# kabachuha/sd-webui-text2video

Measured on AMD Instinct MI355X. Metric: denoised frames/sec (UNet+VAE), ModelScope 24f@256x256, higher is better.
Workload: dtype f16; 1 GPU; ModelScope t2v fp16 (random-init 1.41B UNetSD + VAE decoder), 24 frames @ 256x256, 50 DDIM_Gaussian steps, CFG 9.0 (BASELINE.json configs[1]); one step = one whole video; frames_per_video=24, videos_per_batch=1, layout=single, layout_requested=auto, parallelism=1 GPU: cond+uncond batched as b=2

## Files before the change

sd-webui-text2video_amd/csrc/executor.hip:

```cpp
#include <hip/hip_runtime.h>

#include <cstdio>
#include <cstdlib>
#include <cstring>
#include <initializer_list>
#include <string>
#include <type_traits>
#include <vector>

#include "t2v_kernels.h"

namespace {

thread_local std::string g_err;

int fail(int code, const std::string& msg) {
  g_err = msg;
  return code;
}

inline bool resolve_ptrs(t2v_op& op, const uint64_t* ext, int n_ext) {
  for (int k = 0; k < T2V_OP_NP; ++k) {
    const uint64_t v = op.p[k];
    if (v != 0 && v < T2V_EXT_SLOTS) {
      if ((int)v >= n_ext || ext == nullptr) return false;
      op.p[k] = ext[v];
    }
  }
  return true;
}

enum GemmForm {
  GEMM_MALFORMED,
  GEMM_PLAIN, GEMM_GEGLU,
  GEMM_STATS,
  GEMM_LN_ROW, GEMM_LN_CROSS,
  GEMM_GN_TILE, GEMM_GN_SPLITK,
  GEMM_TATTN, GEMM_XATTN,
};
inline bool gemm_writes_gn(GemmForm f) { return f == GEMM_GN_TILE || f == GEMM_GN_SPLITK; }
struct GemmView {
  GemmForm form;
  const char* why;
  const t2v_tile* tile;
  int M, N, K, lda, ldw, ldc, ldr, ldrb;
  int gather, epi, act, out_dtype, out_item, split, bias_m, halo, rows_per_batch;
  int Hin, Win, Cin, stride, up, Hout, Wout, F, HW, tpix;
  int ln_mode, ld_ln;
  int hilo, out_lo;
  int res_wrap, a_wrap;
  int64_t n_out;
  int gn_rows, ld_gn, gn_silu, gn_lo, gn_groups, gn_skip_out;
  int xa_ldk, xa_lc, xa_lcp, xa_k_sample, xa_vt_sample;
  float ln_eps, attn_scale, gn_eps;
  bool waive_min_m;
  uint64_t A, W, bias, rowbias, ln_gb, res, out, ws;
  uint64_t tickets, ln_out, stats;
  uint64_t gn_gb, gn_out, xa_k, xa_vt;
  uint64_t scratch, barrier;
};

GemmView gemm_decode(const t2v_op& op) {
  const int32_t* I = op.i;
  const uint64_t* P = op.p;
  GemmView v;
  memset(&v, 0, sizeof v);
  const int M = v.M = I[0], N = v.N = I[1], K = v.K = I[2], g = v.gather = I[7], epi = v.epi = I[16];
  const bool plain = g == T2V_GATHER_PLAIN, conv = g == T2V_GATHER_CONV3X3 || g == T2V_GATHER_CONV3X3_C8;
  v.lda = I[3]; v.ldw = I[4]; v.ldc = I[5]; v.ldr = I[6]; v.ldrb = I[21];
  v.act = I[18]; v.out_dtype = I[17]; v.out_item = I[17] == T2V_F32 ? 4 : 2; v.split = I[19] > 1 ? I[19] : 1; v.bias_m = I[20]; v.halo = I[23];
  v.rows_per_batch = I[15] > 0 ? I[15] : 1;
  if (g == T2V_GATHER_TCONV3 || (plain && epi == T2V_EPI_TATTN)) { v.F = I[8]; v.HW = I[9]; }
  else { v.Hin = I[8]; v.Win = I[9]; }
  if (plain && epi == T2V_EPI_TATTN) v.tpix = I[10]; else v.Cin = I[10];
  v.stride = I[11]; v.up = I[12]; v.Hout = I[13]; v.Wout = I[14];
  if (plain) { v.ln_mode = I[8]; v.ld_ln = I[9]; v.hilo = I[11]; v.out_lo = I[11] == 1; }
  if (plain && epi != T2V_EPI_TATTN) { v.res_wrap = I[12]; v.a_wrap = I[13]; }
  if (I[30] > 0) v.res_wrap = I[30];
  v.n_out = epi == T2V_EPI_GEGLU ? N / 2 : N;
  if (epi == T2V_EPI_XATTN) { v.xa_ldk = I[24]; v.xa_lc = I[25]; v.xa_lcp = I[26]; v.xa_k_sample = I[27]; v.xa_vt_sample = I[28]; v.xa_k = P[8]; v.xa_vt = P[9]; }
  else { v.gn_rows = I[24]; v.ld_gn = I[25]; v.gn_silu = I[26]; v.gn_lo = I[27]; v.gn_groups = I[28]; v.gn_skip_out = I[29]; v.gn_gb = P[8]; v.gn_out = P[9]; }
  v.ln_eps = op.f[0]; v.attn_scale = op.f[1]; v.gn_eps = op.f[2];
  v.waive_min_m = I[31] == 1;
  const bool ln = plain && epi != T2V_EPI_TATTN && (I[8] == 1 || I[8] == 2);
  v.form = epi == T2V_EPI_TATTN ? GEMM_TATTN : epi == T2V_EPI_XATTN ? GEMM_XATTN : epi == T2V_EPI_GN ? (v.split > 1 ? GEMM_GN_SPLITK : GEMM_GN_TILE)
         : epi == T2V_EPI_GEGLU ? GEMM_GEGLU : epi == T2V_EPI_STATS ? GEMM_STATS : !ln ? GEMM_PLAIN : I[8] == 1 ? GEMM_LN_ROW : GEMM_LN_CROSS;
  v.A = P[0]; v.W = P[1]; v.bias = P[2]; v.res = P[4]; v.out = P[5]; v.ws = P[6]; v.scratch = P[10]; v.barrier = P[11];
  (ln ? v.ln_gb : v.rowbias) = P[3];
  (ln ? v.ln_out : v.form == GEMM_STATS ? v.stats : v.tickets) = P[7];

  auto bad = [&](const char* why) { v.form = GEMM_MALFORMED; v.why = why; return v; };
  if (M <= 0 || N <= 0 || K <= 0) return bad("empty GEMM");
  if (N % 4 != 0) return bad("N must be a multiple of 4");
  if (K % 8 != 0 || v.lda % 8 != 0 || v.ldw % 8 != 0) return bad("K, lda, ldw must be multiples of 8");
  if (v.ldc % 4 != 0) return bad("ldc must be a multiple of 4");
  if (g == T2V_GATHER_CONV3X3 || g == T2V_GATHER_TCONV3) {
    if (v.Cin % 64 != 0) return bad("conv Cin must be a multiple of 64");
    if (K != (g == T2V_GATHER_CONV3X3 ? 9 : 3) * v.Cin) return bad("K != taps*Cin");
  } else if (g == T2V_GATHER_CONV3X3_C8) {
    if (v.Cin != 8 || K != 72 || v.lda != 8) return bad("C8 conv needs Cin == lda == 8, K == 72");
  } else if (!plain) {
    return bad("unknown gather mode");
  }
  if (conv) {
    if (v.stride != 1 && v.stride != 2) return bad("stride must be 1 or 2");
    if (v.up != 0 && v.up != 1) return bad("upsample must be 0 or 1");
    if (v.Hout <= 0 || v.Wout <= 0 || M % (v.Hout * v.Wout) != 0) return bad("M not a multiple of Hout*Wout");
  }
  if (g == T2V_GATHER_TCONV3 && (v.F <= 0 || v.HW <= 0 || M % (v.F * v.HW) != 0)) return bad("M not a multiple of F*HW");
  if (epi == T2V_EPI_GEGLU && (N % 32 != 0 || v.out_dtype != T2V_F16)) return bad("GEGLU needs N % 32 == 0, fp16 out");
  if (epi == T2V_EPI_STATS && (P[7] == 0 || v.split > 1 || v.ln_mode == 1))
    return bad("column statistics (T2V_EPI_STATS): strips pointer p[7], no split-K, no fused LayerNorm");
  if (epi < 0 || epi > T2V_EPI_XATTN) return bad("unknown epilogue");
  if (v.act < 0 || v.act > 2) return bad("unknown activation (0 none, 1 SiLU, 2 ReLU)");
  const t2v_tile* tile = v.tile = t2v_tile_of(I[22]);
  if (tile == nullptr) return bad("unknown tile id");
  if (I[30] != 0) {
    if (I[30] < 0 || M > 2 * I[30] || v.res == 0) return bad("residual row wrap i[30]: positive, M <= 2 * wrap, and a residual");
    if (epi == T2V_EPI_GEGLU || epi == T2V_EPI_TATTN || epi == T2V_EPI_XATTN || (plain && (I[12] != 0 || v.ln_mode != 0)))
      return bad("residual row wrap i[30]: plain / statistics / GroupNorm epilogues only, not beside i[12] or a fused LayerNorm");
  }
  if (epi == T2V_EPI_XATTN) {
    if (!plain || N % 64 != 0 || K % 64 != 0 || v.out_dtype != T2V_F16 || v.split > 1 || v.act != 0 || v.ln_mode != 0 || v.out_lo)
      return bad("fused cross-attention: plain gather, N = 64 * heads, K % 64 == 0, fp16 out, no split-K / activation / LayerNorm / hi + lo output");
    if (!t2v_tile_fuses(tile, T2V_TILE_XATTN, N)) return bad("fused cross-attention: tile 8 / 11 with N == 320, or tile 0 / 5 with N % 128 == 0");
    if (v.bias != 0 || P[3] != 0 || v.res != 0 || v.xa_k == 0 || v.xa_vt == 0 || !(v.attn_scale > 0.f)) return bad("fused cross-attention: no bias / row bias / residual; K, V^T and a positive scale are required");
    if (v.xa_lc < 1 || v.xa_lc > 96 || v.xa_ldk < N || v.xa_ldk % 8 != 0 || v.xa_lcp < ((v.xa_lc + 31) / 32) * 32 || v.xa_lcp % 8 != 0 || I[15] <= 0 || I[15] % 32 != 0 || v.xa_k_sample < 0 || v.xa_vt_sample < 0)
      return bad("fused cross-attention: 1 .. 96 keys, ld(K) >= N, V^T rows of >= ceil32(keys) halfs, rows per sample a multiple of 32");
    if (v.ldc < N || v.ldc % 4 != 0) return bad("fused cross-attention: ldc");
    if (I[12] != 0) return bad("fused cross-attention: no residual wrap");
    return v;
  }
  if (epi == T2V_EPI_GN) {
    const int rows = v.gn_rows, groups = v.gn_groups, bm = tile->bm, bn = tile->bn;
    if (g == T2V_GATHER_CONV3X3_C8 || (g == T2V_GATHER_CONV3X3 && v.up != 0)) return bad("fused GroupNorm: not for the C8 stem / the upsampling gather");
    if (v.bias_m != 0 || K % 64 != 0 || v.act != 0) return bad("fused GroupNorm: no bias along M, no activation, K % 64 == 0");
    if (plain && (v.ln_mode != 0 || v.out_lo)) return bad("fused GroupNorm: no fused LayerNorm / hi + lo output on the same op");
    if (groups <= 0 || N % groups != 0 || rows <= 0 || M % rows != 0) return bad("fused GroupNorm: N % groups == 0, rows per instance must divide M");
    if (v.split > 1) {
      if (groups > 32 || N % 8 != 0 || N / 8 > 512 || v.ws == 0) return bad("fused GroupNorm on a split-K GEMM: groups <= 32, N % 8 == 0, N <= 4096, a slab workspace");
    } else {
      if (!tile->has(T2V_TILE_GN)) return bad("fused GroupNorm: tile must be 8, 11, 3, 5 or 0");
      if (!t2v_tile_fuses(tile, T2V_TILE_GN, N)) return bad("fused GroupNorm on the 128x128-class kernel: N % 128 == 0");
      if (N / groups > bn || (bn + N / groups - 1) / (N / groups) + 1 > T2V_GN_PIECES) return bad("fused GroupNorm: a group no wider than the tile");
      if (rows % 32 != 0 || !(rows >= bm || 2 * rows == bm))
        return bad("fused GroupNorm: rows per instance must be a multiple of 32 and >= the tile's rows (or exactly half of them): at most two instances per row tile");
    }
    if (v.gn_gb == 0 || v.gn_out == 0 || v.scratch == 0 || v.barrier == 0) return bad("fused GroupNorm: gamma|beta, output, scratch and barrier words are required");
    if (v.ld_gn < N * (v.gn_lo ? 2 : 1) || v.ld_gn % 4 != 0) return bad("fused GroupNorm: leading dimension of the normalised output");
    if (v.gn_skip_out == 0 && v.out == 0) return bad("fused GroupNorm: `out` is null but i[29] asks for it");
    if (v.ldc < N || (v.res != 0 && (v.ldr < N || v.ldr % 4 != 0))) return bad("fused GroupNorm: ldc / ldr must be >= N and multiples of 4");
  }
  if (v.split > 1 && v.ws == 0) return bad("split-K without workspace");
  if (P[3] != 0 && I[15] <= 0 && !(v.ln_mode == 1 || v.ln_mode == 2)) return bad("rowbias without rows_per_batch");
  if ((epi == T2V_EPI_TATTN) != tile->has(T2V_TILE_TATTN_ONLY)) return bad("tile 10 is the fused QKV + temporal attention tile (T2V_EPI_TATTN), and only that");
  if (epi == T2V_EPI_TATTN) {
    const int F = v.F, HW = v.HW, tpix = v.tpix;
    if (!plain || N % 192 != 0 || K % 64 != 0 || v.out_dtype != T2V_F16 || v.split > 1 || v.act != 0)
      return bad("fused temporal attention: plain gather, N = 192 * heads, K % 64 == 0, fp16 out, no split-K / activation");
    if (F < 2 || F > 32 || HW < 1 || tpix < 1 || tpix > 12 || tpix * F > 192) return bad("fused temporal attention: 2 <= F <= 32, 1 <= pixels per tile <= 12, pixels * F <= 192");
    const int tiles_ps = (HW + tpix - 1) / tpix;
    if (M % 192 != 0 || (M / 192) % tiles_ps != 0) return bad("fused temporal attention: M must be samples * ceil(HW / pixels per tile) * 192");
    if (v.bias != 0 || P[3] != 0 || v.res != 0 || v.A == 0 || v.W == 0 || v.out == 0 || !(v.attn_scale > 0.f))
      return bad("fused temporal attention: no bias / row bias / residual; A, W, out and a positive scale are required");
    if (v.ldc < (N / 192) * 64 || v.ldc % 4 != 0) return bad("fused temporal attention: ldc < heads * 64");
    return v;
// ... 141 lines not shown
      if (axis != 0 && axis != 1) return bad("resample: axis must be 0 (horizontal) or 1 (vertical)");
      if (form < 0 || form > 2) return bad("resample: unknown output form (0 uint8, 1 fp32 tokens, 2 fp16 tokens)");
      if (form != 0 && (ld < 3 || op.p[4] == 0)) return bad("resample: the token forms need ld >= 3 and the 256-entry value table p[4]");
      if (op.p[0] == 0 || op.p[1] == 0 || op.p[2] == 0 || op.p[3] == 0) return bad("null resample pointer (source, destination, coefficients, bounds)");
      const long row_px = axis == 0 ? out : op.i[2];
      if (row_px > (1 << 28)) return bad("resample: row too long");
      if (grid.rows * grid.tiles > 0xffffffL) return bad("resample: too many rows for one launch (rows x tiles of 256 units <= 2^24 - 1)");
      return 0;
    }
    case T2V_OP_DEPTH_TOKENS:
      if (op.i[0] <= 0 || op.i[1] <= 0 || op.i[2] <= 0 || op.i[1] % 8 != 0 || op.i[2] % 8 != 0) return bad("depth tokens: frames > 0, H and W positive multiples of 8");
      if ((long)op.i[1] * op.i[2] > (1L << 28)) return bad("depth tokens: frame too large");
      if ((op.i[3] != T2V_F16 && op.i[3] != T2V_F32) || (op.i[4] != 0 && op.i[4] != 1) || op.i[5] < 64 || op.i[5] % 8 != 0)
        return bad("depth tokens: input dtype, normalise flag (0 | 1), ld_out >= 64 and a multiple of 8");
      if (op.p[0] == 0 || op.p[1] == 0) return bad("null depth-token pointer");
      if (op.p[1] >= T2V_EXT_SLOTS && op.p[1] % 16 != 0) return bad("depth tokens: the output must be 16-byte aligned");
      return 0;
    case T2V_OP_AVGPOOL2:
      if (op.i[0] <= 0 || op.i[1] < 2 || op.i[2] < 2 || op.i[3] <= 0 || op.i[3] % 4 != 0) return bad("average pooling: images > 0, H and W >= 2, C % 4 == 0");
      if (op.i[4] < op.i[3] || op.i[4] % 4 != 0) return bad("average pooling: ld_in >= C and a multiple of 4");
      if (op.p[0] == 0 || (op.p[1] == 0 && op.p[2] == 0)) return bad("average pooling: an input and at least one output");
      if ((op.p[1] != 0 && (op.i[5] < op.i[3] || op.i[5] % 4 != 0)) || (op.p[2] != 0 && (op.i[6] < op.i[3] || op.i[6] % 4 != 0)))
        return bad("average pooling: output leading dimensions >= C and multiples of 4");
      return 0;
    case T2V_OP_EMPHASIS:
      if (op.i[0] <= 0 || op.i[1] <= 0 || op.i[1] % 4 != 0 || (long)op.i[0] * op.i[1] > (1L << 28)) return bad("emphasis: rows > 0, W a positive multiple of 4, rows * W <= 2^28");
      if (op.i[2] < op.i[1] || op.i[3] < op.i[1] || op.i[3] % 4 != 0 || (op.i[4] != T2V_F16 && op.i[4] != T2V_F32))
        return bad("emphasis: leading dimensions >= W (the output's a multiple of 4), input dtype fp16 | fp32");
      if (op.p[0] == 0 || op.p[1] == 0 || op.p[2] == 0) return bad("null emphasis pointer");
      if (op.p[2] >= T2V_EXT_SLOTS && op.p[2] % 16 != 0) return bad("emphasis: the output must be 16-byte aligned");
      return 0;
    case T2V_OP_FINGERPRINT:
      if (op.i[0] <= 0 || op.i[1] < op.i[0]) return bad("fingerprint: n segments > 0, at least one chunk per segment");
      if (op.p[0] == 0 || op.p[1] == 0 || op.p[2] == 0) return bad("null fingerprint pointer");
      for (int k = 0; k < 3; ++k)
        if (op.p[k] >= T2V_EXT_SLOTS && op.p[k] % 8 != 0) return bad("fingerprint: the tables and the output must be 8-byte aligned");
      return 0;
    case T2V_OP_LORA_MERGE:
      if (op.i[0] <= 0 || op.i[1] < op.i[0]) return bad("lora merge: n segments > 0, at least one tile per segment");
      if (op.p[0] == 0 || op.p[1] == 0) return bad("null lora merge pointer");
      for (int k = 0; k < 2; ++k)
        if (op.p[k] >= T2V_EXT_SLOTS && op.p[k] % 8 != 0) return bad("lora merge: the tables must be 8-byte aligned");
      return 0;
    case T2V_OP_FREEU: {
      const t2v_freeu_view v = t2v_freeu_decode(op);
      return v.ok ? 0 : bad(v.why);
    }
    case T2V_OP_ALLGATHER:
      if (op.i[2] < 1 || op.i[3] < 0 || op.i[3] >= op.i[2] || op.p[0] == 0) return bad("bad all-gather record");
      return 0;
    case T2V_OP_HALO_EXCHANGE:
      if (op.i[2] < 1 || op.p[0] == 0 || op.i[3] < -1 || op.i[4] < -1) return bad("bad halo-exchange record");
      return 0;
    case T2V_OP_STATS_HALO:
      if (op.i[2] < 1 || op.i[3] < 0 || op.i[3] >= op.i[2] || op.p[0] == 0 || op.p[1] == 0) return bad("bad statistics + halo record");
      if (op.i[6] < 1 || op.i[7] < -1 || op.i[8] < -1 || op.i[7] >= op.i[2] || op.i[8] >= op.i[2]) return bad("bad statistics + halo neighbours");
      return 0;
    case T2V_OP_RESHARD_ROWS:
      if (op.i[0] <= 0 || op.i[1] <= 0 || op.i[2] <= 0 || op.i[3] < 0 || op.i[4] < 0) return bad("bad row-resharding shape");
      if (op.i[5] < op.i[1] || op.i[6] < op.i[1] || op.p[0] == 0 || op.p[1] == 0) return bad("row resharding: leading dimension / pointer");
      if (op.p[2] != 0 && op.i[7] != T2V_F32) return bad("row resharding: the residual form is fp32");
      if (op.i[9] > 1 && (op.i[9] > 64 || op.i[10] < 0 || op.i[11] < 0 || op.i[12] < 0 || op.i[13] < -1 || op.i[13] >= op.i[9] ||
                          (op.i[14] != 0 && op.i[14] != 1) || (op.i[13] >= 0 && op.p[3] == 0)))
        return bad("row resharding: bad multi-part record (parts, part strides, own part)");
      return 0;
    case T2V_OP_ALLTOALL:
      if (op.i[2] < 1 || op.i[3] < 0 || op.i[3] >= op.i[2] || op.i[4] < 1 || op.i[5] < 1 || op.i[5] > op.i[4]) return bad("bad all-to-all record");
      if ((op.i[6] != 0 && op.i[6] != 1) || op.p[0] == 0 || op.p[1] == 0) return bad("bad all-to-all direction / pointer");
      return 0;
    default:
      return bad("unknown op kind");
  }
}

GemmParams gemm_params(const GemmView& v) {
  GemmParams p;
  memset(&p, 0, sizeof p);
  p.M = v.M; p.N = v.N; p.K = v.K;
  p.lda = v.lda; p.ldw = v.ldw; p.ldc = v.ldc; p.ldr = v.ldr; p.ldrb = v.ldrb;
  p.gather = v.gather;
  p.Hin = v.Hin; p.Win = v.Win; p.Cin = v.Cin; p.stride = v.stride; p.up = v.up; p.Hout = v.Hout; p.Wout = v.Wout; p.F = v.F; p.HW = v.HW;
  p.rows_per_batch = v.rows_per_batch;
  p.epi = v.form == GEMM_GEGLU || v.form == GEMM_TATTN ? v.epi : T2V_EPI_NONE;
  p.out_f32 = v.out_dtype == T2V_F32; p.act = v.act; p.splitk = v.split; p.bias_m = v.bias_m; p.halo = v.halo;
  auto ptr = [](auto& dst, uint64_t a) { dst = reinterpret_cast<std::remove_reference_t<decltype(dst)>>(a); };
  ptr(p.A, v.A); ptr(p.W, v.W); ptr(p.bias, v.bias); ptr(p.rowbias, v.rowbias); ptr(p.res, v.res); ptr(p.out, v.out); ptr(p.ws, v.ws); ptr(p.stats, v.stats);
  if (v.split > 1) ptr(p.tickets, v.tickets);
  p.out_lo = v.out_lo; p.res_wrap = v.res_wrap; p.a_wrap = v.a_wrap;
  const bool gn = gemm_writes_gn(v.form), ln = v.form == GEMM_LN_ROW || v.form == GEMM_LN_CROSS;
  if (gn) {
    ptr(p.gn_gb, v.gn_gb); ptr(p.gn_out, v.gn_out);
    p.gn_rows = v.gn_rows; p.ld_gn = v.ld_gn; p.gn_silu = v.gn_silu; p.gn_lo = v.gn_lo ? v.N : 0;
    p.gn_cpg = v.N / v.gn_groups; p.gn_store_out = v.gn_skip_out ? 0 : 1; p.gn_eps = v.gn_eps;
  }
  if (ln) {
    ptr(p.ln_gb, v.ln_gb); ptr(p.ln_out, v.ln_out);
    p.ld_ln = v.ld_ln; p.ln_eps = v.ln_eps; p.ln_x = v.form == GEMM_LN_CROSS;
  }
  if (gn || v.form == GEMM_LN_CROSS) {
    ptr(p.gn_part, v.scratch); ptr(p.gn_bar, v.barrier);
    p.gn_fault = t2v_coop_fault_word();
    t2v_exchange_ids(&p.gn_seq, &p.gn_want);
  }
  if (v.form == GEMM_XATTN) {
    ptr(p.xa_k, v.xa_k); ptr(p.xa_vt, v.xa_vt);
    p.xa_ldk = v.xa_ldk; p.xa_lc = v.xa_lc; p.xa_lcp = v.xa_lcp; p.xa_k_sample = v.xa_k_sample; p.xa_vt_sample = v.xa_vt_sample;
  }
  if (v.form == GEMM_TATTN) { p.tpix = v.tpix; p.tiles_ps = (v.HW + v.tpix - 1) / v.tpix; }
  if (v.form == GEMM_TATTN || v.form == GEMM_XATTN) p.attn_scale_log2 = v.attn_scale * 1.44269504088896340736f;
  return p;
}
hipError_t launch_op(const t2v_op& op, hipStream_t s) {
  switch (op.kind) {
    case T2V_OP_GEMM: {
      const GemmView v = gemm_decode(op);
      if (v.form == GEMM_MALFORMED) return hipErrorInvalidValue;
      const bool gemm2 = v.form == GEMM_TATTN || (v.tile->has(T2V_TILE_GEMM2) && v.gather != T2V_GATHER_CONV3X3_C8 && v.K % 64 == 0);
      return gemm2 ? t2v_launch_gemm2(gemm_params(v), v.tile->id, s) : t2v_launch_gemm(gemm_params(v), s);
    }
    case T2V_OP_GROUPNORM: return t2v_launch_groupnorm(op, s);
    case T2V_OP_LAYERNORM: return t2v_launch_layernorm(op, s);
    case T2V_OP_ATTENTION: return t2v_launch_attention(op, s);
    case T2V_OP_SOFTMAX: return t2v_launch_softmax(op, s);
    case T2V_OP_NCTHW_TO_CL: return t2v_launch_ncthw_to_cl(op, s);
    case T2V_OP_CL_TO_NCTHW: return t2v_launch_cl_to_ncthw(op, s);
    case T2V_OP_TIME_EMBED: return t2v_launch_time_embed(op, s);
    case T2V_OP_COPY2D: return t2v_launch_copy2d(op, s);
    case T2V_OP_DDIM_STEP: return t2v_launch_ddim_step(op, s);
    case T2V_OP_LINCOMB: return t2v_launch_lincomb(op, s);
    case T2V_OP_RELPOS_ATTN: return t2v_launch_relpos_attention(op, s);
    case T2V_OP_EMBED_ROWS: return t2v_launch_embed_rows(op, s);
    case T2V_OP_TO_UINT8: return t2v_launch_to_uint8(op, s);
    case T2V_OP_RESAMPLE: return t2v_launch_resample(op, s);
    case T2V_OP_RESHARD_ROWS: return t2v_launch_reshard_rows(op, s);
    case T2V_OP_DEPTH_TOKENS: return t2v_launch_depth_tokens(op, s);
    case T2V_OP_AVGPOOL2: return t2v_launch_avgpool2(op, s);
    case T2V_OP_EMPHASIS: return t2v_launch_emphasis(op, s);
    case T2V_OP_FINGERPRINT: return t2v_launch_fingerprint(op, s);
    case T2V_OP_LORA_MERGE: return t2v_launch_lora_merge(op, s);
    case T2V_OP_FREEU: return t2v_launch_freeu(op, s);
    case T2V_OP_MEMSET: {
      const size_t bytes = (size_t)(uint32_t)op.i[0] | ((size_t)(uint32_t)op.i[1] << 32);
      return hipMemsetAsync(reinterpret_cast<void*>(op.p[0]), 0, bytes, s);
    }
    default: return hipErrorInvalidValue;
  }
}

constexpr int FF_FUSE_DEFAULT = 1;
constexpr int FF_MIN_M_DEFAULT = 49152;
bool ff_fuse_enabled() {
  static int mode = -1;
  if (mode < 0) {
    const char* e = getenv("T2V_FF_FUSE");
    mode = e != nullptr ? (strcmp(e, "0") != 0 ? 1 : 0) : FF_FUSE_DEFAULT;
  }
  return mode == 1;
}
int ff_min_m() {
  static int min_m = -1;
  if (min_m < 0) {
    const char* e = getenv("T2V_FF_FUSE_MIN_M");
    const long v = e != nullptr ? atol(e) : 0;
    min_m = v > 0 && v < (1L << 30) ? (int)v : FF_MIN_M_DEFAULT;
  }
  return min_m;
}
// ... 573 lines not shown
```

sd-webui-text2video_amd/csrc/gemm2.hip:

```cpp
#include "t2v_kernels.h"

namespace {

__device__ __attribute__((aligned(256))) unsigned char g2_zero_page[256];

constexpr int G_CONV_UP = 100;

template <int N>
__device__ __forceinline__ void wait_vmcnt() {
  asm volatile("s_waitcnt vmcnt(%0)" ::"n"(N) : "memory");
}

template <int WM, int WN, int TM, int TN, int BK, int STAGES, int MINW, int GATHER, int XE = T2V_XE_NONE, bool TAT = false>
__global__ __launch_bounds__(WM * WN * 64, MINW) void gemm2_kernel(const GemmParams p) {
  constexpr int NW = WM * WN;
  constexpr int BM = WM * TM * 32, BN = WN * TN * 32;
  constexpr int ROW_BYTES = BK * 2;
  constexpr int RPS = 1024 / ROW_BYTES;
  constexpr int CPR = BK / 8;
  constexpr int XSLABS = BM / RPS, WSLABS = BN / RPS;
  static_assert(XSLABS % NW == 0, "token slabs must divide evenly over the waves");
  constexpr int XPW = XSLABS / NW;
  constexpr int WPW = (WSLABS + NW - 1) / NW;
  constexpr int LPS = XPW + WPW;
  constexpr int STAGE_BYTES = (XSLABS + WSLABS) * 1024;
  constexpr int DUMMY_OFF = STAGES * STAGE_BYTES;
  static_assert(LPS * (STAGES - 1) < 64, "vmcnt is a 6-bit counter");

  extern __shared__ __attribute__((aligned(16))) unsigned char smem[];

  const int tid = threadIdx.x;
  const int lane = tid & 63;
  const int wave = __builtin_amdgcn_readfirstlane(tid >> 6);
  const int wm = wave / WN, wn = wave % WN;

  const int tiles_n = (p.N + BN - 1) / BN;
  const int tiles_m = (p.M - p.m_begin + BM - 1) / BM;
  int tile_m, tile_n;
  t2v_tile_of_block(blockIdx.x, tiles_m, tiles_n, p.panel, tile_m, tile_n);
  const int m0 = p.m_begin + tile_m * BM, n0 = tile_n * BN;

  const int KT = (p.K + BK - 1) / BK;
  const int kt_begin = blockIdx.y * p.kt_per_split;
  const int kt_end = min(KT, kt_begin + p.kt_per_split);
  const int nkt = kt_end - kt_begin;

  const unsigned char* zero = g2_zero_page;

  const int lrow = lane / CPR;
  const int pchunk = lane % CPR;
  auto swz = [](int r) { return BK == 64 ? ((r >> 1) & 7) : ((r >> 2) & 3); };
  constexpr int STEP = BK * 2;

  constexpr int TAPS = (GATHER == T2V_GATHER_CONV3X3 || GATHER == G_CONV_UP) ? 9 : (GATHER == T2V_GATHER_TCONV3 ? 3 : 1);
  constexpr bool general = GATHER == G_CONV_UP;
  const unsigned char* xptr[XPW];
  int xstep[XPW];
  unsigned xmask[XPW];
  long xoff[general ? XPW : 1];
  int xy[general ? XPW : 1], xx[general ? XPW : 1];
  auto xrow0 = [&](int j) { return (wave + j * NW) * RPS; };
  auto wrow0 = [&](int j) { return (wave + j * NW) * RPS; };
#pragma unroll
  for (int j = 0; j < XPW; ++j) {
    const int r = xrow0(j) + lrow;
    const int m = m0 + r;
    const int lc = pchunk ^ swz(r);
    const bool valid = m < p.M;
    xmask[j] = 0; xstep[j] = 0;
    xptr[j] = zero;
    if (GATHER == T2V_GATHER_PLAIN) {
      if constexpr (TAT) {
        const int pl = r / p.F, f = r - pl * p.F;
        const int smp = tile_m / p.tiles_ps, pix = (tile_m - smp * p.tiles_ps) * p.tpix + pl;
        if (pl < p.tpix && pix < p.HW) {
          const long mm = ((long)smp * p.F + f) * p.HW + pix;
          xptr[j] = reinterpret_cast<const unsigned char*>(p.A + mm * p.lda + (long)kt_begin * BK + lc * 8);
          xstep[j] = STEP;
        }
      } else if (valid) {
        const int ma = (p.a_wrap && m >= p.a_wrap) ? m - p.a_wrap : m;
        xptr[j] = reinterpret_cast<const unsigned char*>(p.A + (long)ma * p.lda + (long)kt_begin * BK + lc * 8);
// ... 255 lines not shown
          }
      }
    }
    return;
  }
  if (p.epi == T2V_EPI_NONE) {
    __builtin_amdgcn_s_barrier();
    if constexpr (XE == T2V_XE_GN) {
      t2v_epilogue_rows_gn<WM, WN, TM, TN>(p, acc, smem, lane, wave, m0, n0, tile_m, tile_n, tiles_m, tiles_n);
      return;
    }
    if constexpr (XE == T2V_XE_XATTN) {
      t2v_epilogue_xattn<WM, WN, TM, TN>(p, acc, smem, lane, wave, m0, n0);
      return;
    }
    if constexpr (XE == T2V_XE_LNX) {
      t2v_epilogue_rows_lnx<WM, WN, TM, TN>(p, acc, smem, lane, wave, m0, n0, tile_m, tile_n, tiles_n);
      return;
    }
    if constexpr (XE == T2V_XE_LN) {
      float* fs = reinterpret_cast<float*>(smem);
#pragma unroll
      for (int tm = 0; tm < TM; ++tm) {
        if (tm > 0) __syncthreads();
        t2v_epilogue_rows_ln<TN>(p, reinterpret_cast<f32x16 (&)[1][TN]>(acc[tm]), fs + wave * (32 * T2V_EPI_SP), fs + NW * (32 * T2V_EPI_SP), lane, wave,
                                 m0 + (wm * TM + tm) * 32, n0 + wn * TN * 32);
      }
      return;
    }
    t2v_epilogue_rows<TM, TN>(p, acc, reinterpret_cast<float*>(smem) + wave * (32 * T2V_EPI_SP), lane, m0 + wm * TM * 32,
                              n0 + wn * TN * 32, blockIdx.y, tile_m * tiles_n + tile_n);
    return;
  }
  const int mlane = lane & 31, nhalf = (lane >> 5) * 4;
  if (p.epi == T2V_EPI_GEGLU && p.splitk == 1) {
    constexpr int PITCH = TN * 32 + 16;
    constexpr int CPRW = TN * 2;
    __builtin_amdgcn_s_barrier();
    unsigned char* strip = smem + wave * (32 * PITCH);
    const int nw = n0 + wn * TN * 32;
#pragma unroll
    for (int a = 0; a < TM; ++a) {
      const int mt = m0 + (wm * TM + a) * 32;
      if (mt >= p.M) continue;
#pragma unroll
      for (int b = 0; b < TN; ++b) {
        const int nt = nw + b * 32;
#pragma unroll
        for (int qq = 0; qq < 2; ++qq) {
          const int n_val = nt + 16 * qq + nhalf;
          f16x4 o = {(f16)0.f, (f16)0.f, (f16)0.f, (f16)0.f};
          if (n_val < p.N) {
            float bv[4] = {0, 0, 0, 0}, bg[4] = {0, 0, 0, 0};
            if (p.bias) {
              const f32x4 ba = *reinterpret_cast<const f32x4*>(p.bias + n_val);
              const f32x4 bb = *reinterpret_cast<const f32x4*>(p.bias + n_val + 8);
#pragma unroll
              for (int r = 0; r < 4; ++r) { bv[r] = ba[r]; bg[r] = bb[r]; }
            }
#pragma unroll
            for (int r = 0; r < 4; ++r) o[r] = (f16)((acc[a][b][8 * qq + r] + bv[r]) * t2v_gelu_erf(acc[a][b][8 * qq + 4 + r] + bg[r]));
          }
          *reinterpret_cast<f16x4*>(strip + mlane * PITCH + (b * 16 + 8 * qq + nhalf) * 2) = o;
        }
      }
      __builtin_amdgcn_fence(__ATOMIC_RELEASE, "wavefront");
      const int c_out0 = nw >> 1;
#pragma unroll
      for (int u = lane; u < 32 * CPRW; u += 64) {
        const int row = u / CPRW, ch = u - row * CPRW;
        const int m = mt + row, c = c_out0 + ch * 8;
        if (m < p.M && c < (p.N >> 1)) {
          const f16x8 v = *reinterpret_cast<const f16x8*>(strip + row * PITCH + ch * 16);
          *reinterpret_cast<f16x8*>(reinterpret_cast<f16*>(p.out) + (size_t)m * p.ldc + c) = v;
        }
      }
      __builtin_amdgcn_fence(__ATOMIC_RELEASE, "wavefront");
    }
    return;
  }
  t2v_store_splitk_slab<TM, TN>(p, acc, lane, m0 + wm * TM * 32, n0 + wn * TN * 32, blockIdx.y);
}

template <int WM, int WN, int TM, int TN, int BK, int STAGES, int MINW, int GATHER, int XE = T2V_XE_NONE, bool TAT = false>
hipError_t launch_cfg_gather(const GemmParams& p, hipStream_t s) {
  constexpr int BM = WM * TM * 32, BN = WN * TN * 32;
  constexpr int ring = STAGES * (BM + BN) * BK * 2 + 1024;
  constexpr int gn_lds = t2v_gn_epilogue_lds(WM * WN, WM * TM, BN);
  constexpr int lnx_lds = t2v_lnx_epilogue_lds(WM * WN, WN, BM);
  constexpr int xa_lds = t2v_xattn_epilogue_lds(BM, BN);
  constexpr int lds = TAT ? (BM * 272 + 12 * 64 * 72 > ring ? BM * 272 + 12 * 64 * 72 : ring)
                          : (XE == T2V_XE_GN && gn_lds > ring ? gn_lds : (XE == T2V_XE_LNX && lnx_lds > ring ? lnx_lds : (XE == T2V_XE_XATTN && xa_lds > ring ? xa_lds : ring)));
  const int tiles_n = (p.N + BN - 1) / BN;
  const int tiles = ((p.M - p.m_begin + BM - 1) / BM) * tiles_n;
  auto k = gemm2_kernel<WM, WN, TM, TN, BK, STAGES, MINW, GATHER, XE, TAT>;
  static t2v_device_flags attr_set;
  {
    const hipError_t e = t2v_set_dynamic_lds(reinterpret_cast<const void*>(k), lds, attr_set, s);
    if (e != hipSuccess) return e;
  }
  if constexpr (XE == T2V_XE_GN || XE == T2V_XE_LNX) {
    static int occ[T2V_MAX_DEVICES] = {};
    if (p.splitk != 1 || !t2v_coop_allowed()) return hipErrorCooperativeLaunchTooLarge;
    const long cap = t2v_grid_capacity(reinterpret_cast<const void*>(k), WM * WN * 64, lds, s, occ);
    return t2v_launch_coresident(p, BM, tiles_n, cap, XE == T2V_XE_GN ? t2v_lcm(BM, p.gn_rows) : BM, XE == T2V_XE_GN ? 2 * T2V_GN_PIECES * 16 : BM * 16,
                                 [&](const GemmParams& q, int nwg) {
      hipLaunchKernelGGL(k, dim3(nwg, 1), dim3(WM * WN * 64), lds, s, q);
      return hipGetLastError();
    });
  }
  hipLaunchKernelGGL(k, dim3(tiles, p.splitk > 1 ? p.splitk : 1), dim3(WM * WN * 64), lds, s, p);
  return hipGetLastError();
}

template <int TILE, int WM, int WN, int TM, int TN, int BK, int STAGES, int MINW>
hipError_t launch_cfg(const GemmParams& pin, hipStream_t s) {
  constexpr t2v_tile T = *t2v_tile_of(TILE);
  static_assert(T.has(T2V_TILE_GEMM2) && T.bm == WM * TM * 32 && T.bn == WN * TN * 32 && T.waves == WM * WN, "the configuration is not the table's tile");
  GemmParams p = pin;
  if (p.epi != T2V_EPI_NONE && p.epi != T2V_EPI_GEGLU && !(p.epi == T2V_EPI_TATTN && p.gather == T2V_GATHER_PLAIN)) return hipErrorInvalidValue;
  {
    const int tiles_m = (p.M + T.bm - 1) / T.bm, tiles_n = (p.N + T.bn - 1) / T.bn;
    p.panel = t2v_choose_panel(p, tiles_m, tiles_n);
    t2v_normalize_splitk(p, BK, (long)tiles_m * tiles_n);
  }
  const bool gn_here = p.gn_out != nullptr && p.splitk == 1;
  if (gn_here && (!T.has(T2V_TILE_GN) || (p.gather == T2V_GATHER_CONV3X3 && p.up))) return hipErrorInvalidValue;
  if (p.ln_x && (!T.has(T2V_TILE_LNX) || p.gather != T2V_GATHER_PLAIN)) return hipErrorInvalidValue;
  hipError_t e;
  switch (p.gather) {
    case T2V_GATHER_PLAIN:
      if constexpr (T.has(T2V_TILE_TATTN_ONLY)) {
        if (p.epi != T2V_EPI_TATTN || p.splitk != 1 || p.tpix < 1 || p.tpix > 12 || p.tpix * p.F > T.bm || p.F > 32) return hipErrorInvalidValue;
        e = launch_cfg_gather<WM, WN, TM, TN, BK, STAGES, MINW, T2V_GATHER_PLAIN, T2V_XE_NONE, true>(p, s);
        break;
      }
      if (p.epi == T2V_EPI_TATTN) return hipErrorInvalidValue;
      if constexpr (T.has(T2V_TILE_XATTN)) {
        if (p.xa_k != nullptr) {
          e = launch_cfg_gather<WM, WN, TM, TN, BK, STAGES, MINW, T2V_GATHER_PLAIN, T2V_XE_XATTN>(p, s);
          break;
        }
      }
      if (p.xa_k != nullptr) return hipErrorInvalidValue;
      if constexpr (T.has(T2V_TILE_LN)) {
        if (p.ln_out != nullptr) {
          e = launch_cfg_gather<WM, WN, TM, TN, BK, STAGES, MINW, T2V_GATHER_PLAIN, T2V_XE_LN>(p, s);
          break;
        }
      }
      if constexpr (T.has(T2V_TILE_GN)) {
        if (gn_here) { e = launch_cfg_gather<WM, WN, TM, TN, BK, STAGES, MINW, T2V_GATHER_PLAIN, T2V_XE_GN>(p, s); break; }
      }
      if constexpr (T.has(T2V_TILE_LNX)) {
        if (p.ln_x) { e = launch_cfg_gather<WM, WN, TM, TN, BK, STAGES, MINW, T2V_GATHER_PLAIN, T2V_XE_LNX>(p, s); break; }
      }
      e = launch_cfg_gather<WM, WN, TM, TN, BK, STAGES, MINW, T2V_GATHER_PLAIN>(p, s);
      break;
    case T2V_GATHER_CONV3X3:
      if constexpr (T.has(T2V_TILE_GN)) {
        if (gn_here && !p.up) { e = launch_cfg_gather<WM, WN, TM, TN, BK, STAGES, MINW, T2V_GATHER_CONV3X3, T2V_XE_GN>(p, s); break; }
      }
      if (p.up) e = launch_cfg_gather<WM, WN, TM, TN, BK, STAGES, MINW, G_CONV_UP>(p, s);
      else e = launch_cfg_gather<WM, WN, TM, TN, BK, STAGES, MINW, T2V_GATHER_CONV3X3>(p, s);
      break;
    case T2V_GATHER_TCONV3:
      if constexpr (T.has(T2V_TILE_GN)) {
        if (gn_here) { e = launch_cfg_gather<WM, WN, TM, TN, BK, STAGES, MINW, T2V_GATHER_TCONV3, T2V_XE_GN>(p, s); break; }
      }
      e = launch_cfg_gather<WM, WN, TM, TN, BK, STAGES, MINW, T2V_GATHER_TCONV3>(p, s);
      break;
    default: return hipErrorInvalidValue;
  }
  if (e != hipSuccess) return e;
  if (p.splitk > 1 && p.tickets == nullptr) e = p.gn_out != nullptr ? t2v_launch_splitk_reduce_gn(p, s) : t2v_launch_splitk_reduce(p, s);
  return e;
}

constexpr int FF_C = 320, FF_HID = 1280, FF_BM = 192, FF_CH = 64, FF_NCHUNK = FF_HID / FF_CH, FF_KT1 = FF_C / 64, FF_TPC = FF_KT1 + 1;
constexpr int FF_NW = 12, FF_SLOT = 40 * 1024, FF_STAGES = 3, FF_LPS = 4;
constexpr int FF_W1_OFF = FF_BM * 128;
constexpr int FF_HP = FF_CH * 2 + 16;
constexpr int FF_H_OFF = FF_STAGES * FF_SLOT, FF_B_OFF = FF_H_OFF + FF_BM * FF_HP, FF_DUMMY_OFF = FF_B_OFF + 2 * FF_HID * 4;
constexpr int FF_LDS = FF_DUMMY_OFF + 1024;
static_assert(FF_NW * 32 * T2V_EPI_SP * 4 <= FF_H_OFF, "the epilogue strips alias the ring");

__global__ __launch_bounds__(FF_NW * 64, 3) void ff_fused_kernel(const GemmParams p1, const GemmParams p2) {
  extern __shared__ __attribute__((aligned(16))) unsigned char smem[];
  const int tid = threadIdx.x;
  const int lane = tid & 63;
  const int wave = __builtin_amdgcn_readfirstlane(tid >> 6);
  const int wm = wave >> 1, wn = wave & 1;
  const int m0 = blockIdx.x * FF_BM;

  float* b1s = reinterpret_cast<float*>(smem + FF_B_OFF);
  for (int i = tid; i < 2 * FF_HID; i += FF_NW * 64) b1s[i] = p1.bias ? p1.bias[i] : 0.f;

  const int lrow = lane >> 3, pchunk = lane & 7;
  auto swz = [](int r) { return (r >> 1) & 7; };
  const bool last_real = wave < 4;
  unsigned xoffs[2];
#pragma unroll
  for (int j = 0; j < 2; ++j) {
    const int r = (wave + FF_NW * j) * 8 + lrow;
    xoffs[j] = (min(m0 + r, p1.M - 1) * p1.lda + (pchunk ^ swz(r)) * 8) * 2;
  }
  const int wr0 = wave * 8 + lrow, wlc = (pchunk ^ swz(wr0)) * 8;
  const unsigned w1off = (wr0 * p1.ldw + wlc) * 2, w2off = (wr0 * p2.ldw + wlc) * 2;
  const int w1step = 96 * p1.ldw * 2, w2step = 96 * p2.ldw * 2;
  const unsigned char* xb = reinterpret_cast<const unsigned char*>(p1.A);
  const unsigned char* w1b = reinterpret_cast<const unsigned char*>(p1.W);
  const unsigned char* w2b = reinterpret_cast<const unsigned char*>(p2.W);
  const long w1chunk = (long)(2 * FF_CH) * p1.ldw * 2;
  auto stage_piece = [&](int slot, int sc, int sk, int j) {
    unsigned char* dst = smem + slot * FF_SLOT + (wave + FF_NW * j) * 1024;
    const int scl = min(sc, FF_NCHUNK - 1);
    const bool dummy = j == 3 && !last_real;
    const int jj = dummy ? 0 : j;
    const unsigned char* base;
    unsigned off;
    if (sk == FF_KT1) { base = w2b + (scl * (FF_CH * 2) + jj * w2step); off = w2off; }
    else if (jj < 2) { base = xb + sk * 128; off = xoffs[jj]; }
    else { base = w1b + (scl * w1chunk + sk * 128 + (jj - 2) * w1step); off = w1off; }
    if (dummy) dst = smem + FF_DUMMY_OFF;
    asm volatile("" : "+s"(base));
    const unsigned char* src = base + (size_t)off;
    t2v_glds16(src, dst);
  };

  f32x16 acc2[1][5], acc1[2];
#pragma unroll
  for (int b = 0; b < 5; ++b)
#pragma unroll
    for (int r = 0; r < 16; ++r) acc2[0][b][r] = 0.f;

#pragma unroll
  for (int g = 0; g < FF_STAGES - 1; ++g)
#pragma unroll
    for (int j = 0; j < FF_LPS; ++j) stage_piece(g, 0, g, j);

  const int frow = lane & 31, fhalf = lane >> 5;
  const int fsw = swz(frow) << 4;
// ... 106 lines not shown
```

sd-webui-text2video_amd/csrc/t2v_kernels.h:

```cpp
#pragma once
#include <hip/hip_runtime.h>
#include <stdint.h>

#include <string>

#include "../../include/t2v_hip.h"

typedef _Float16 f16;
typedef f16 f16x4 __attribute__((ext_vector_type(4)));
typedef f16 f16x8 __attribute__((ext_vector_type(8)));
typedef float f32x4 __attribute__((ext_vector_type(4)));
typedef float f32x8 __attribute__((ext_vector_type(8)));
typedef float f32x16 __attribute__((ext_vector_type(16)));

struct GemmParams {
  const f16* A;
  const f16* W;
  const float* bias;
  const float* rowbias;
  const float* res;
  void* out;
  float* ws;
  int M, N, K;
  int m_begin;
  int lda, ldw, ldc, ldr, ldrb;
  int gather;
  int Hin, Win, Cin, stride, up, Hout, Wout;
  int F, HW;
  int rows_per_batch;
  int epi, out_f32, act, splitk, bias_m;
  int kt_per_split;
  int halo;
  int panel;
  const float* ln_gb;
  f16* ln_out;
  int ld_ln;
  float ln_eps;
  int tpix, tiles_ps;
  float attn_scale_log2;
  int* tickets;
  int out_lo;
  float* stats;
  int a_wrap, res_wrap;
  const float* gn_gb;
  f16* gn_out;
  double* gn_part;
  unsigned* gn_bar;
  unsigned* gn_fault;
  int ld_gn, gn_rows, gn_cpg, gn_silu, gn_lo, gn_store_out;
  float gn_eps;
  int ln_x;
  unsigned gn_seq, gn_want;
  const f16* xa_k;
  const f16* xa_vt;
  int xa_ldk, xa_lc, xa_lcp, xa_k_sample, xa_vt_sample;
};


#if defined(__HIP_DEVICE_COMPILE__) && !defined(__gfx950__) && !defined(__gfx942__)
#error "libt2v_hip is written for gfx950 (MI355X); the device-scope exchange helpers assume gfx94x / gfx950 memory semantics"
#endif

__device__ __forceinline__ void t2v_st_dev(float* p, f32x4 v) { asm volatile("global_store_dwordx4 %0, %1, off sc1" ::"v"(p), "v"(v) : "memory"); }
__device__ __forceinline__ f32x4 t2v_ld_dev(const float* p) {
  f32x4 v;
  asm volatile("global_load_dwordx4 %0, %1, off sc1" : "=&v"(v) : "v"(p) : "memory");
  return v;
}
__device__ __forceinline__ void t2v_wait_dev(f32x4& a, f32x4& b, f32x4& c, f32x4& d) {
  asm volatile("s_waitcnt vmcnt(0)" : "+v"(a), "+v"(b), "+v"(c), "+v"(d)::"memory");
}
__device__ __forceinline__ void t2v_wait_vm0() { asm volatile("s_waitcnt vmcnt(0)" ::: "memory"); }

__device__ __forceinline__ void t2v_tile_of_block(int b, int tiles_m, int tiles_n, int pw, int& tile_m, int& tile_n) {
  const int ntiles = tiles_m * tiles_n;
  const int q = ntiles >> 3, r = ntiles & 7, xcd = b & 7, j = b >> 3;
  const int lin = (xcd < r ? xcd * (q + 1) : r * (q + 1) + (xcd - r) * q) + j;
  const int per_panel = tiles_m * pw;
  const int pnl = lin / per_panel, rem = lin - pnl * per_panel;
  const int n_start = pnl * pw;
  const int w_here = min(pw, tiles_n - n_start);
  tile_m = rem / w_here;
  tile_n = n_start + rem - tile_m * w_here;
}

inline int t2v_choose_panel(const GemmParams& p, int tiles_m, int tiles_n) {
  const double a_rows = p.gather == T2V_GATHER_CONV3X3 ? (double)p.M * p.stride * p.stride / (p.up ? 4.0 : 1.0) : (double)p.M;
  const double Ab = a_rows * (p.gather == T2V_GATHER_PLAIN ? p.K : p.Cin) * 2.0;
  const double Wb = (double)p.N * p.K * 2.0;
  int best_xn = 1;
  double best = 1e300;
  for (int xn = 1; xn <= 8 && xn <= tiles_n; ++xn) {
    const double cost = xn * Ab + (8.0 / xn) * Wb;
    if (cost < best) { best = cost; best_xn = xn; }
  }
  return (tiles_n + best_xn - 1) / best_xn;
}

constexpr int T2V_MAX_DEVICES = 64;
inline int t2v_device_of(hipStream_t s) {
  int d = 0;
  hipDevice_t sd;
  if (s != nullptr && hipStreamGetDevice(s, &sd) == hipSuccess) d = (int)sd;
  else (void)hipGetDevice(&d);
  return (d >= 0 && d < T2V_MAX_DEVICES) ? d : 0;
}
struct t2v_device_flags { bool set[T2V_MAX_DEVICES] = {}; };
inline hipError_t t2v_set_dynamic_lds(const void* kernel, int lds_bytes, t2v_device_flags& flags, hipStream_t s) {
  const int d = t2v_device_of(s);
  if (flags.set[d]) return hipSuccess;
  const hipError_t e = hipFuncSetAttribute(kernel, hipFuncAttributeMaxDynamicSharedMemorySize, lds_bytes);
  if (e == hipSuccess) flags.set[d] = true;
  return e;
}
int t2v_num_cus(hipStream_t s);
struct t2v_device_guard {
// ... 1035 lines not shown
```

Baseline: 18.93 frames/s.

## Add halo-staged 3x3 conv GEMM kernel that reuses one input slab across taps

Adds a new 3x3 stride-1 conv implicit-GEMM kernel. Per 64-channel chunk it stages a single halo window of input rows (the tile plus padding) into LDS and reads all nine taps from it with row shifts and a per-row validity mask. The old path re-gathers the input once per tap. Input loads are double-buffered, weight slabs are ring-buffered, and the global loads are spread across the MFMA loop with hand-counted vmcnt waits. It is enabled by default for eligible small-width convs on selected tile configs, with an env opt-out and a legacy flag. In exchange it uses more LDS, which may lower occupancy, and it depends on a delicate wait schedule.

```diff
diff --git a/sd-webui-text2video_amd/csrc/executor.hip b/sd-webui-text2video_amd/csrc/executor.hip
--- a/sd-webui-text2video_amd/csrc/executor.hip
+++ b/sd-webui-text2video_amd/csrc/executor.hip
@@ -54,6 +54,7 @@
   int xa_ldk, xa_lc, xa_lcp, xa_k_sample, xa_vt_sample;
   float ln_eps, attn_scale, gn_eps;
   bool waive_min_m;
+  bool conv_legacy;
   uint64_t A, W, bias, rowbias, ln_gb, res, out, ws;
   uint64_t tickets, ln_out, stats;
   uint64_t gn_gb, gn_out, xa_k, xa_vt;
@@ -82,6 +83,7 @@
   else { v.gn_rows = I[24]; v.ld_gn = I[25]; v.gn_silu = I[26]; v.gn_lo = I[27]; v.gn_groups = I[28]; v.gn_skip_out = I[29]; v.gn_gb = P[8]; v.gn_out = P[9]; }
   v.ln_eps = op.f[0]; v.attn_scale = op.f[1]; v.gn_eps = op.f[2];
   v.waive_min_m = I[31] == 1;
+  v.conv_legacy = g == T2V_GATHER_CONV3X3 && I[31] == 1;
   const bool ln = plain && epi != T2V_EPI_TATTN && (I[8] == 1 || I[8] == 2);
   v.form = epi == T2V_EPI_TATTN ? GEMM_TATTN : epi == T2V_EPI_XATTN ? GEMM_XATTN : epi == T2V_EPI_GN ? (v.split > 1 ? GEMM_GN_SPLITK : GEMM_GN_TILE)
          : epi == T2V_EPI_GEGLU ? GEMM_GEGLU : epi == T2V_EPI_STATS ? GEMM_STATS : !ln ? GEMM_PLAIN : I[8] == 1 ? GEMM_LN_ROW : GEMM_LN_CROSS;
@@ -389,7 +391,7 @@
   p.Hin = v.Hin; p.Win = v.Win; p.Cin = v.Cin; p.stride = v.stride; p.up = v.up; p.Hout = v.Hout; p.Wout = v.Wout; p.F = v.F; p.HW = v.HW;
   p.rows_per_batch = v.rows_per_batch;
   p.epi = v.form == GEMM_GEGLU || v.form == GEMM_TATTN ? v.epi : T2V_EPI_NONE;
-  p.out_f32 = v.out_dtype == T2V_F32; p.act = v.act; p.splitk = v.split; p.bias_m = v.bias_m; p.halo = v.halo;
+  p.out_f32 = v.out_dtype == T2V_F32; p.act = v.act; p.splitk = v.split; p.bias_m = v.bias_m; p.halo = v.halo; p.conv_legacy = v.conv_legacy;
   auto ptr = [](auto& dst, uint64_t a) { dst = reinterpret_cast<std::remove_reference_t<decltype(dst)>>(a); };
   ptr(p.A, v.A); ptr(p.W, v.W); ptr(p.bias, v.bias); ptr(p.rowbias, v.rowbias); ptr(p.res, v.res); ptr(p.out, v.out); ptr(p.ws, v.ws); ptr(p.stats, v.stats);
   if (v.split > 1) ptr(p.tickets, v.tickets);
diff --git a/sd-webui-text2video_amd/csrc/gemm2.hip b/sd-webui-text2video_amd/csrc/gemm2.hip
--- a/sd-webui-text2video_amd/csrc/gemm2.hip
+++ b/sd-webui-text2video_amd/csrc/gemm2.hip
@@ -1,3 +1,7 @@
+#include <cstdlib>
+#include <cstring>
+#include <type_traits>
+
 #include "t2v_kernels.h"
 
 namespace {
@@ -419,10 +423,219 @@
   t2v_store_splitk_slab<TM, TN>(p, acc, lane, m0 + wm * TM * 32, n0 + wn * TN * 32, blockIdx.y);
 }
 
-template <int WM, int WN, int TM, int TN, int BK, int STAGES, int MINW, int GATHER, int XE = T2V_XE_NONE, bool TAT = false>
+template <int NW, int BM, int BN, int STAGES>
+struct halo_geom {
+  static constexpr int PAD = 40;
+  static constexpr int HROWS = BM + 2 * PAD, HSLABS = HROWS / 8, HPW = (HSLABS + NW - 1) / NW, HBYTES = HROWS * 128;
+  static constexpr int WSLABS = BN / 8, WPW = (WSLABS + NW - 1) / NW, WSLOT = BN * 128;
+  static constexpr int W_OFF = 2 * HBYTES, DUMMY_OFF = W_OFF + STAGES * WSLOT, ZERO_OFF = DUMMY_OFF + 1024, LDS = ZERO_OFF + 128;
+  static constexpr int HTAPS = 11 - STAGES;
+  static constexpr int tap_of(int i) { return (i * HTAPS) / HPW; }
+  static constexpr int count(int tap) { int n = 0; for (int i = 0; i < HPW; ++i) n += tap_of(i) == tap; return n; }
+  static constexpr int first(int tap) { int n = 0; for (int i = 0; i < HPW; ++i) n += tap_of(i) < tap; return n; }
+  static constexpr int wait_at(int tap) { int n = 0; for (int d = 1; d <= STAGES - 2; ++d) n += WPW + count((tap + 9 - d) % 9); return n; }
+  static_assert(STAGES >= 2 && STAGES <= 4 && HROWS % 8 == 0 && tap_of(HPW - 1) < HTAPS, "halo schedule");
+  static_assert(HPW + (STAGES - 1) * WPW + WPW + HPW < 64, "vmcnt is a 6-bit counter");
+  static_assert(LDS <= 160 * 1024, "LDS");
+};
+
+template <int WM, int WN, int TM, int TN, int STAGES, int MINW, int XE = T2V_XE_NONE>
+__global__ __launch_bounds__(WM * WN * 64, MINW) void gemm2_halo_kernel(const GemmParams p) {
+  constexpr int NW = WM * WN;
+  constexpr int BM = WM * TM * 32, BN = WN * TN * 32;
+  using HG = halo_geom<NW, BM, BN, STAGES>;
+  constexpr int HPW = HG::HPW, WPW = HG::WPW;
+
+  extern __shared__ __attribute__((aligned(16))) unsigned char smem[];
+
+  const int tid = threadIdx.x;
+  const int lane = tid & 63;
+  const int wave = __builtin_amdgcn_readfirstlane(tid >> 6);
+  const int wm = wave / WN, wn = wave % WN;
+
+  const int tiles_n = (p.N + BN - 1) / BN;
+  const int tiles_m = (p.M - p.m_begin + BM - 1) / BM;
+  int tile_m, tile_n;
+  t2v_tile_of_block(blockIdx.x, tiles_m, tiles_n, p.panel, tile_m, tile_n);
+  const int m0 = p.m_begin + tile_m * BM, n0 = tile_n * BN;
+
+  const int KT = p.K / 64;
+  const int kt_begin = blockIdx.y * p.kt_per_split;
+  const int nkt = min(KT, kt_begin + p.kt_per_split) - kt_begin;
+  const int nch = nkt / 9;
+
+  const unsigned char* zero = g2_zero_page;
+  if (tid < 32) reinterpret_cast<int*>(smem + HG::ZERO_OFF)[tid] = 0;
+  asm volatile("s_waitcnt lgkmcnt(0)" ::: "memory");
+
+  const int lrow = lane >> 3, pchunk = lane & 7;
+  auto swz = [](int r) { return (r >> 1) & 7; };
+  const int hw = p.Hin * p.Win;
+  const long a_rows = (long)((p.M + hw - 1) / hw) * hw;
+  unsigned hoff[HPW];
+#pragma unroll
+  for (int i = 0; i < HPW; ++i) {
+    const int h = (wave + i * NW) * 8 + lrow;
+    const long g = min(max((long)m0 - HG::PAD + h, 0L), a_rows - 1);
+    hoff[i] = (unsigned)(g * p.lda * 2) + (unsigned)((pchunk ^ swz(h)) * 16);
+  }
+  const unsigned char* hnext = reinterpret_cast<const unsigned char*>(p.A) + (long)(kt_begin / 9) * 128;
+  const unsigned char* wptr[WPW];
+  unsigned wok = 0;
+#pragma unroll
+  for (int j = 0; j < WPW; ++j) {
+    const int sl = wave + j * NW, r = sl * 8 + lrow;
+    const int n = n0 + r;
+    const bool ok = sl < HG::WSLABS && n < p.N;
+    wptr[j] = ok ? reinterpret_cast<const unsigned char*>(p.W + (size_t)n * p.ldw + kt_begin * 64 + (pchunk ^ swz(r)) * 8) : zero;
+    wok |= (ok ? 1u : 0u) << j;
+  }
+  auto stage_h = [&](int buf, int i) {
+    const int sl = wave + i * NW;
+    unsigned char* dst = ((i + 1) * NW <= HG::HSLABS || sl < HG::HSLABS) ? smem + buf + sl * 1024 : smem + HG::DUMMY_OFF;
+    const unsigned char* base = hnext;
+    asm volatile("" : "+s"(base));
+    t2v_glds16(base + (size_t)hoff[i], dst);
+  };
+  auto stage_w = [&](int fs, int j, bool live) {
+    const int sl = wave + j * NW;
+    unsigned char* dst = ((j + 1) * NW <= HG::WSLABS || sl < HG::WSLABS) ? smem + HG::W_OFF + fs * HG::WSLOT + sl * 1024 : smem + HG::DUMMY_OFF;
+    const void* src = live ? wptr[j] : zero;
+    wptr[j] += ((wok >> j) & 1u) << 7;
+    t2v_glds16(src, dst);
+  };
+
+  f32x16 acc[TM][TN];
+#pragma unroll
+  for (int a = 0; a < TM; ++a)
+#pragma unroll
+    for (int b = 0; b < TN; ++b)
+#pragma unroll
+      for (int r = 0; r < 16; ++r) acc[a][b][r] = 0.f;
+
+#pragma unroll
+  for (int i = 0; i < HPW; ++i) stage_h(0, i);
+  if (nch > 1) hnext += 128;
+#pragma unroll
+  for (int g = 0; g < STAGES - 1; ++g)
+#pragma unroll
+    for (int j = 0; j < WPW; ++j) stage_w(g, j, true);
+
+  const int frow = lane & 31, fhalf = lane >> 5;
+  int hrow[TM];
+  unsigned fmask[TM];
+#pragma unroll
+  for (int a = 0; a < TM; ++a) {
+    const int r = (wm * TM + a) * 32 + frow;
+    const int m = m0 + r;
+    hrow[a] = r + HG::PAD;
+    const int img = m / hw, rem = m - img * hw;
+    const int yo = rem / p.Win, xo = rem - yo * p.Win;
+    fmask[a] = 0;
+    for (int t = 0; t < 9; ++t) {
+      const int yv = yo + t / 3 - 1, xv = xo + t % 3 - 1;
+      if (m < p.M && yv >= 0 && yv < p.Hin && xv >= 0 && xv < p.Win) fmask[a] |= 1u << t;
+    }
+  }
+  const int wb0 = (wn * TN * 32 + frow) * 128, wsw = swz(frow) << 4;
+
+  int slot = 0;
+  auto tap_body = [&](auto tap_c, int c, int hcur) {
+    constexpr int tap = decltype(tap_c)::value;
+    wait_vmcnt<HG::wait_at(tap)>();
+    __builtin_amdgcn_s_barrier();
+    asm volatile("" ::: "memory");
+    int fs = slot + STAGES - 1;
+    if (fs >= STAGES) fs -= STAGES;
+    const bool wlive = c * 9 + tap + STAGES - 1 < nkt;
+    int shift = (tap / 3 - 1) * p.Win + (tap % 3 - 1);
+    asm volatile("" : "+s"(shift));
+    int xb[TM], xs[TM];
+#pragma unroll
+    for (int a = 0; a < TM; ++a) {
+      const int h = hrow[a] + shift;
+      unsigned fm = fmask[a];
+      asm volatile("" : "+v"(fm));
+      const bool on = (fm >> tap) & 1u;
+      xb[a] = on ? hcur + h * 128 : HG::ZERO_OFF;
+      xs[a] = on ? swz(h) << 4 : 0;
+    }
+    const unsigned char* st = smem + HG::W_OFF + slot * HG::WSLOT + wb0;
+#pragma unroll
+    for (int kk = 0; kk < 4; ++kk) {
+      const int lc4 = (kk * 2 + fhalf) << 4;
+      f16x8 xf[TM], wf[TN];
+#pragma unroll
+      for (int a = 0; a < TM; ++a) xf[a] = *reinterpret_cast<const f16x8*>(smem + xb[a] + (lc4 ^ xs[a]));
+#pragma unroll
+      for (int b = 0; b < TN; ++b) wf[b] = *reinterpret_cast<const f16x8*>(st + b * 4096 + (lc4 ^ wsw));
+      constexpr int NH = HG::count(tap), H0 = HG::first(tap), NP = NH + WPW;
+      constexpr int SPREAD = STAGES == 2 ? 2 : 4;
+      if (kk < SPREAD) {
+#pragma unroll
+        for (int q = (NP * kk) / SPREAD; q < (NP * (kk + 1)) / SPREAD; ++q) {
+          if (q < NH) stage_h(HG::HBYTES - hcur, H0 + q);
+          else stage_w(fs, q - NH, wlive);
+        }
+      }
+#pragma unroll
+      for (int a = 0; a < TM; ++a)
+#pragma unroll
+        for (int b = 0; b < TN; ++b)
+          acc[a][b] = __builtin_amdgcn_mfma_f32_32x32x16_f16(wf[b], xf[a], acc[a][b], 0, 0, 0);
+    }
+    slot = slot + 1 == STAGES ? 0 : slot + 1;
+  };
+  int hcur = 0;
+  for (int c = 0; c < nch; ++c) {
+    tap_body(std::integral_constant<int, 0>{}, c, hcur);
+    tap_body(std::integral_constant<int, 1>{}, c, hcur);
+    tap_body(std::integral_constant<int, 2>{}, c, hcur);
+    tap_body(std::integral_constant<int, 3>{}, c, hcur);
+    tap_body(std::integral_constant<int, 4>{}, c, hcur);
+    tap_body(std::integral_constant<int, 5>{}, c, hcur);
+    tap_body(std::integral_constant<int, 6>{}, c, hcur);
+    tap_body(std::integral_constant<int, 7>{}, c, hcur);
+    tap_body(std::integral_constant<int, 8>{}, c, hcur);
+    hcur = HG::HBYTES - hcur;
+    if (c + 2 < nch) hnext += 128;
+  }
+  wait_vmcnt<0>();
+
+  __builtin_amdgcn_s_barrier();
+  if constexpr (XE == T2V_XE_GN) {
+    t2v_epilogue_rows_gn<WM, WN, TM, TN>(p, acc, smem, lane, wave, m0, n0, tile_m, tile_n, tiles_m, tiles_n);
+    return;
+  }
+  t2v_epilogue_rows<TM, TN>(p, acc, reinterpret_cast<float*>(smem) + wave * (32 * T2V_EPI_SP), lane, m0 + wm * TM * 32,
+                            n0 + wn * TN * 32, blockIdx.y, tile_m * tiles_n + tile_n);
+}
+
+constexpr bool conv_halo_tile(int tile) { return tile == 1 || tile == 3 || tile == 5 || tile == 8 || tile == 9 || tile == 11; }
+constexpr int CONV_HALO_DEFAULT = 1;
+bool conv_halo_enabled() {
+  static int mode = -1;
+  if (mode < 0) {
+    const char* e = getenv("T2V_CONV_HALO");
+    mode = e != nullptr ? (strcmp(e, "0") != 0 ? 1 : 0) : CONV_HALO_DEFAULT;
+  }
+  return mode == 1;
+}
+bool conv_halo_eligible(const GemmParams& p) {
+  return conv_halo_enabled() && !p.conv_legacy && p.gather == T2V_GATHER_CONV3X3 && p.epi == T2V_EPI_NONE && p.stride == 1 && p.up == 0 &&
+         p.halo == 0 && p.a_wrap == 0 && p.Hin == p.Hout && p.Win == p.Wout && p.Win >= 1 && p.Win <= 32 && p.Hin >= 1 && p.Cin % 64 == 0 &&
+         p.K == 9 * p.Cin && (p.splitk == 1 || p.kt_per_split % 9 == 0) &&
+         ((long)p.M + (long)p.Hin * p.Win) * p.lda * 2 < (1L << 31);
+}
+
+template <int WM, int WN, int TM, int TN, int BK, int STAGES, int MINW, int GATHER, int XE = T2V_XE_NONE, bool TAT = false, bool HALO = false>
 hipError_t launch_cfg_gather(const GemmParams& p, hipStream_t s) {
   constexpr int BM = WM * TM * 32, BN = WN * TN * 32;
-  constexpr int ring = STAGES * (BM + BN) * BK * 2 + 1024;
+  static_assert(!HALO || (GATHER == T2V_GATHER_CONV3X3 && BK == 64 && !TAT), "the halo staging is a form of the 3x3 gather");
+  constexpr int ring = [] {
+    if constexpr (HALO) return halo_geom<WM * WN, BM, BN, STAGES>::LDS;
+    else return STAGES * (BM + BN) * BK * 2 + 1024;
+  }();
   constexpr int gn_lds = t2v_gn_epilogue_lds(WM * WN, WM * TM, BN);
   constexpr int lnx_lds = t2v_lnx_epilogue_lds(WM * WN, WN, BM);
   constexpr int xa_lds = t2v_xattn_epilogue_lds(BM, BN);
@@ -430,7 +643,10 @@
                           : (XE == T2V_XE_GN && gn_lds > ring ? gn_lds : (XE == T2V_XE_LNX && lnx_lds > ring ? lnx_lds : (XE == T2V_XE_XATTN && xa_lds > ring ? xa_lds : ring)));
   const int tiles_n = (p.N + BN - 1) / BN;
   const int tiles = ((p.M - p.m_begin + BM - 1) / BM) * tiles_n;
-  auto k = gemm2_kernel<WM, WN, TM, TN, BK, STAGES, MINW, GATHER, XE, TAT>;
+  void (*k)(const GemmParams) = [] {
+    if constexpr (HALO) return gemm2_halo_kernel<WM, WN, TM, TN, STAGES, MINW, XE>;
+    else return gemm2_kernel<WM, WN, TM, TN, BK, STAGES, MINW, GATHER, XE, TAT>;
+  }();
   static t2v_device_flags attr_set;
   {
     const hipError_t e = t2v_set_dynamic_lds(reinterpret_cast<const void*>(k), lds, attr_set, s);
@@ -495,6 +711,15 @@
       e = launch_cfg_gather<WM, WN, TM, TN, BK, STAGES, MINW, T2V_GATHER_PLAIN>(p, s);
       break;
     case T2V_GATHER_CONV3X3:
+      if constexpr (conv_halo_tile(TILE)) {
+        if (conv_halo_eligible(p)) {
+          if constexpr (T.has(T2V_TILE_GN)) {
+            if (gn_here) { e = launch_cfg_gather<WM, WN, TM, TN, BK, STAGES, MINW, T2V_GATHER_CONV3X3, T2V_XE_GN, false, true>(p, s); break; }
+          }
+          e = launch_cfg_gather<WM, WN, TM, TN, BK, STAGES, MINW, T2V_GATHER_CONV3X3, T2V_XE_NONE, false, true>(p, s);
+          break;
+        }
+      }
       if constexpr (T.has(T2V_TILE_GN)) {
         if (gn_here && !p.up) { e = launch_cfg_gather<WM, WN, TM, TN, BK, STAGES, MINW, T2V_GATHER_CONV3X3, T2V_XE_GN>(p, s); break; }
       }
diff --git a/sd-webui-text2video_amd/csrc/t2v_kernels.h b/sd-webui-text2video_amd/csrc/t2v_kernels.h
--- a/sd-webui-text2video_amd/csrc/t2v_kernels.h
+++ b/sd-webui-text2video_amd/csrc/t2v_kernels.h
@@ -32,6 +32,7 @@
   int kt_per_split;
   int halo;
   int panel;
+  int conv_legacy;
   const float* ln_gb;
   f16* ln_out;
   int ld_ln;
```

Result: faster. 19.14 frames/s (median of 6 runs) (+1.1%).
